# ADharaUTEXAS123007/PhysicsBasedFWI2

Hardware: AMD Instinct MI355X
Metric: grid-cells*timesteps/sec (forward+adjoint gradient pass) (higher is better)
Workload: dtype f32; 1 GPU; elastic_marmousi2_100x300_32shots_3000steps; shots_per_gpu=32, nt=3000, parallelism=shots x1, kernel_family=forward: single launch, 8 slabs/shot; adjoint: single launch, 8 slabs/shot, snapshots=f32, cells=interior

## Files before the change

physicsbasedfwi2_amd/csrc/mifwi_elastic_cluster.h:

```cpp
#pragma once

constexpr int kEcThreads = 512;
constexpr unsigned kEcMaxSpin = 400000;

struct EcParams {
    int nz, nx, ng, gp, pitch;
    unsigned field_stride;
    long long shot_stride;
    int nshot, NW, PL, shot0, shot1;
    int n_first, n_last;
    int W, wl, xr0, wx, fsurf;
    long long psix_shot, psiz_shot;
    const float *mat, *pz, *px;
    float *fields, *psix, *psiz;
    float *S;
    int s_first;
    long long s_step;
    int nsrc, nrec;
    const int *src_cell;
    const float *src_w, *f;
    const int *rec_cell;
    const float *rec_w;
    float *rec_vx, *rec_vz;
    unsigned long long *xbuf;
    int *err;
    int *xcc_tab;
    int dbg, nap;
    FdK K;
#ifdef MIFWI_ABLATIONS
    long long *trace;
#endif
};

#ifdef MIFWI_ABLATIONS
#define EC_STAMP(k)                                                                                        \
    do {                                                                                                   \
        if (p.trace && tr_on && it >= 64 && it < 128 && (t & 63) == 0)                                     \
            p.trace[((it - 64) * 8 + (t >> 6)) * 16 + (k)] = (long long)__builtin_readcyclecounter();      \
    } while (0)
#define EC_LAGGARD()                                                                                       \
    do {                                                                                                   \
        if ((kDbg(p) & 4096) && w == 1 && s == p.shot0 && (it & 63) == 1)                                  \
            for (int z_ = 0; z_ < 3000; ++z_) __builtin_amdgcn_s_sleep(127);                               \
    } while (0)
#else
#define EC_STAMP(k) do { } while (0)
#define EC_LAGGARD() do { } while (0)
#endif

constexpr int kEcRowFields = 6;
constexpr int kEcGr = 5;

__device__ __forceinline__ int ec_rf_field(int rf) { return (rf == 0 || rf == 3 || rf == 4) ? 1 : 0; }
__device__ __forceinline__ int ec_rf_lds_row(int rf, int R)
{
    return rf == 0 || rf == 1 ? R + 2 : rf == 2 ? R + 3 : rf == 3 ? 0 : 1;
}

__device__ __forceinline__ int ec_opaque(int x)
{
    asm volatile("" : "+v"(x));
    return x;
}
__device__ __forceinline__ unsigned ec_opaque(unsigned x)
{
    asm volatile("" : "+v"(x));
    return x;
}
__device__ __forceinline__ int ec_fresh(int &x)
{
    asm volatile("" : "+v"(x));
    return x;
}
__device__ __forceinline__ unsigned ec_fresh(unsigned &x)
{
    asm volatile("" : "+v"(x));
    return x;
}

__device__ __forceinline__ int ec_su(int x)
{
    x = __builtin_amdgcn_readfirstlane(x);
    asm volatile("" : "+s"(x));
    return x;
}
__device__ __forceinline__ unsigned ec_su(unsigned x) { return (unsigned)ec_su((int)x); }

template <class T>
__device__ __forceinline__ T *ec_at(T *base, unsigned byte_off)
{
    return reinterpret_cast<T *>(reinterpret_cast<char *>(base) + byte_off);
}
template <class T>
__device__ __forceinline__ const T *ec_at(const T *base, unsigned byte_off)
{
    return reinterpret_cast<const T *>(reinterpret_cast<const char *>(base) + byte_off);
}

__device__ __forceinline__ void ec_pin(float4 &a, float4 &b, float4 &c, float4 &d)
{
    asm volatile("" : "+v"(a.x), "+v"(a.y), "+v"(a.z), "+v"(a.w), "+v"(b.x), "+v"(b.y), "+v"(b.z), "+v"(b.w),
                      "+v"(c.x), "+v"(c.y), "+v"(c.z), "+v"(c.w), "+v"(d.x), "+v"(d.y), "+v"(d.z), "+v"(d.w));
}
__device__ __forceinline__ void ec_pin(float4 &a, float4 &b)
{
    asm volatile("" : "+v"(a.x), "+v"(a.y), "+v"(a.z), "+v"(a.w), "+v"(b.x), "+v"(b.y), "+v"(b.z), "+v"(b.w));
}
__device__ __forceinline__ void ec_pin(float2 &a, float2 &b, float2 &c, float2 &d)
{
    asm volatile("" : "+v"(a.x), "+v"(a.y), "+v"(b.x), "+v"(b.y), "+v"(c.x), "+v"(c.y), "+v"(d.x), "+v"(d.y));
}

typedef float ec_f2 __attribute__((ext_vector_type(2)));
__device__ __forceinline__ ec_f2 ec_2(float a, float b) { ec_f2 r; r.x = a; r.y = b; return r; }
__device__ __forceinline__ ec_f2 ec_2(const float4 &v, int h) { return h == 0 ? ec_2(v.x, v.y) : ec_2(v.z, v.w); }
__device__ __forceinline__ ec_f2 dfw2(const FdK &K, ec_f2 fm1, ec_f2 f0, ec_f2 f1, ec_f2 f2)
{
    return __builtin_elementwise_fma(ec_2(K.c1, K.c1), f1 - f0, ec_2(K.c2, K.c2) * (f2 - fm1));
}
__device__ __forceinline__ ec_f2 dbw2(const FdK &K, ec_f2 fm2, ec_f2 fm1, ec_f2 f0, ec_f2 f1)
{
    return __builtin_elementwise_fma(ec_2(K.c1, K.c1), f0 - fm1, ec_2(K.c2, K.c2) * (f1 - fm2));
}

__device__ __forceinline__ void ec_drain_vmem() { __builtin_amdgcn_s_waitcnt(0x0f70); }
__device__ __forceinline__ void ec_settle(float &x) { asm volatile("" : "+v"(x)); }

template <bool AG> struct EcScope { static constexpr int value = AG ? __HIP_MEMORY_SCOPE_AGENT : __HIP_MEMORY_SCOPE_WORKGROUP; };

struct EcHandoff {
    unsigned long long *xw;
    unsigned xslot8;
    int gp, ng, NW, w, R, t;
    int rcv_lo[kEcGr];
    unsigned rcv_off[kEcGr];
    int *err;
    bool failed, no_wait;
    int nap;

    __device__ __forceinline__ void init(unsigned long long *xbuf, int s, int NW_, int w_, int R_, int PL, int gp_,
                                         int ng_, int t_, int *err_, bool no_wait_, int nap_, int plane_a)
    {
        nap = nap_;
        gp = gp_; ng = ng_; NW = NW_; w = w_; R = R_; t = t_; err = err_; failed = false; no_wait = no_wait_;
        xslot8 = 8u * kEcRowFields * gp;
        xw = xbuf + ((long long)s * NW + w) * 4 * (kEcRowFields * gp);
#pragma unroll
        for (int k = 0; k < kEcGr; ++k) {
            const int e = t + k * kEcThreads;
            rcv_lo[k] = -1;
            rcv_off[k] = 4u * xslot8;
            if (e < kEcRowFields * gp) {
                const int cq = e % gp, rf = e / gp;
                const int col = 4 * (cq % ng) + cq / ng;
                const bool from_above = rf >= 3;
                if (cq < 4 * ng && !(from_above ? w == 0 : w == NW - 1)) {
                    rcv_lo[k] = ec_rf_lds_row(rf, R) * PL + 4 + col + (ec_rf_field(rf) ? plane_a : 0);
                    rcv_off[k] = 8u * e + (from_above ? 0u : 8u * xslot8);
                }
            }
        }
    }

    struct Pending {
        const unsigned long long *base;
        unsigned long long v[kEcGr];
        __device__ __forceinline__ void clear()
        {
            base = nullptr;
#pragma unroll
            for (int k = 0; k < kEcGr; ++k) v[k] = 0;
        }
    };
    __device__ __forceinline__ void sweep(Pending &q)
    {
#pragma unroll
        for (int k = 0; k < kEcGr; ++k)
            q.v[k] = __hip_atomic_load(ec_at(q.base, ec_fresh(rcv_off[k])), __ATOMIC_RELAXED, __HIP_MEMORY_SCOPE_AGENT);
    }
    __device__ __forceinline__ void request(Pending &q, int kind, int parity)
    {
        const unsigned xs8 = ec_su(xslot8);
        q.base = ec_at(xw, (unsigned)(kind * 2 + parity) * xs8) - 4 * (xs8 / 8);
        sweep(q);
    }
    template <bool EAGER = false, class Dest>
    __device__ __forceinline__ void complete(Pending &q, unsigned epoch, Dest dest)
    {
        int lo[kEcGr];
        unsigned need[kEcGr];
#pragma unroll
        for (int k = 0; k < kEcGr; ++k) { lo[k] = ec_fresh(rcv_lo[k]); need[k] = ~(unsigned)(lo[k] >> 31); }
        for (unsigned spins = 0;; ++spins) {
            unsigned bad = 0;
#pragma unroll
            for (int k = 0; k < kEcGr; ++k) bad |= ((unsigned)(q.v[k] >> 32) ^ epoch) & need[k];
            if (spins == mifwi::kSlowPollPasses && (t & 63) == 0) atomicAdd(err + mifwi::kErrSlow, 1);
            if (bad == 0 || no_wait || failed) break;
            if (spins > kEcMaxSpin ||
                ((spins & 255u) == 255u && __hip_atomic_load(err, __ATOMIC_RELAXED, __HIP_MEMORY_SCOPE_AGENT))) {
                if (spins > kEcMaxSpin) __hip_atomic_store(err, 1, __ATOMIC_RELAXED, __HIP_MEMORY_SCOPE_AGENT);
                failed = true;
                break;
            }
            if (!(EAGER && spins == 0)) mifwi::poll_nap(nap);
            sweep(q);
        }
#pragma unroll
        for (int k = 0; k < kEcGr; ++k)
            if (lo[k] >= 0) dest(lo[k], __uint_as_float((unsigned)q.v[k]));
        ec_drain_vmem();
    }
    template <class Dest>
    __device__ __forceinline__ void receive(int kind, unsigned epoch, int parity, Dest dest)
    {
        Pending q;
        request(q, kind, parity);
        complete(q, epoch, dest);
    }

    template <bool AG>
    __device__ __forceinline__ void publish(int lrw, int gq, int kind, unsigned epoch, int parity, const float4 &b,
                                            const float4 &a) const
    {
        unsigned long long *x = ec_at(xw, (unsigned)(kind * 2 + parity) * ec_su(xslot8));
        const unsigned long long tag = (unsigned long long)epoch << 32;
        const float bv[4] = {b.x, b.y, b.z, b.w}, av[4] = {a.x, a.y, a.z, a.w};
        const unsigned gp8 = 8u * ec_su((unsigned)gp), ng8 = 8u * ec_su((unsigned)ng), gq8 = 8u * gq;
        auto put = [&](int rf, const float (&v)[4]) {
            unsigned o = rf * gp8 + gq8;
#pragma unroll
            for (int k = 0; k < 4; ++k) {
                __hip_atomic_store(ec_at(x, o), tag | __float_as_uint(v[k]), __ATOMIC_RELAXED, EcScope<AG>::value);
                o = ec_opaque(o + ng8);
            }
        };
        const int wq = ec_su(w), Rq = ec_su(R);
        if (wq > 0) {
            if (lrw == 0) { put(0, av); put(1, bv); }
            if (lrw == 1) put(2, bv);
        }
        if (wq < ec_su(NW) - 1) {
            if (lrw == Rq - 2) put(3, av);
            if (lrw == Rq - 1) { put(4, av); put(5, bv); }
        }
    }
};

#ifndef EC_LATE_INTERIOR
#define EC_LATE_INTERIOR 1
#endif
#ifndef EA_PUBLISH_FIRST
#define EA_PUBLISH_FIRST 1
#endif
#ifndef EA_MATS_AHEAD_A
#define EA_MATS_AHEAD_A 0
#endif
#ifndef EA_MATS_AHEAD_C
#define EA_MATS_AHEAD_C 1
#endif
struct EcSlot { int lrw, g, cls; };
__host__ __device__ __forceinline__ EcSlot ec_slot(int v, int R, int ng, int slots)
{
    EcSlot s;
    s.lrw = 0; s.g = 0; s.cls = 0;
#if EC_LATE_INTERIOR
    const int nint = (R > 4 ? R - 4 : 0) * ng, nb = R * ng - nint;
    int b0 = (nint + 63) & ~63;
    if (b0 + nb > slots) b0 = nint;
    if (v < nint) {
        const int ir = v / ng;
        s.lrw = 2 + ir; s.g = v - ir * ng; s.cls = v < kEcThreads ? 1 : 3;
    } else if (v >= b0 && v < b0 + nb) {
        const int bi = v - b0, br = bi / ng;
        s.g = bi - br * ng;
        s.lrw = (R > 4 && br >= 2) ? R - 4 + br : br;
        s.cls = 2;
    }
#else
    if (v < R * ng) {
        s.lrw = v / ng; s.g = v - s.lrw * ng;
        s.cls = (s.lrw >= 2 && s.lrw < R - 2) ? 1 : 2;
    }
#endif
    return s;
}

constexpr int kNbL = 1, kNbR = 2, kNbFirst = 4, kNbLast = 8;
__host__ __device__ __forceinline__ int ec_nb(int v, int R, int ng, int slots)
{
    const EcSlot s = ec_slot(v, R, ng, slots);
    if (s.cls == 0) return 0;
    const int lane = v & 63;
    const bool lv = lane != 0 && ec_slot(v - 1, R, ng, slots).cls == s.cls;
    const bool rv = lane != 63 && ec_slot(v + 1, R, ng, slots).cls == s.cls;
    return (lv ? kNbL : 0) | (rv ? kNbR : 0) | (s.g == 0 ? kNbFirst : 0) | (s.g == ng - 1 ? kNbLast : 0);
}
inline bool ec_xhalo_deal_ok(int R, int ng, int slots)
{
    for (int v = 0; v < slots; ++v) {
        const EcSlot s = ec_slot(v, R, ng, slots);
        if (s.cls == 0) continue;
        const int nb = ec_nb(v, R, ng, slots), lane = v & 63;
        if (!(nb & (kNbL | kNbR))) return false;
        const int lc = lane != 0 ? ec_slot(v - 1, R, ng, slots).cls : 0;
        if (lc >= 2 && s.cls >= 2 && lc != s.cls) return false;
    }
    return true;
}
__device__ __forceinline__ float ec_lane_below(float old, float x)
{
    return __int_as_float(__builtin_amdgcn_update_dpp(__float_as_int(old), __float_as_int(x), 0x138, 0xf, 0xf, false));
}
__device__ __forceinline__ float ec_lane_above(float old, float x)
{
    return __int_as_float(__builtin_amdgcn_update_dpp(__float_as_int(old), __float_as_int(x), 0x130, 0xf, 0xf, false));
}
__host__ __device__ __forceinline__ int ec_xh_word(int nb, int lo_floats)
{
    const int roff = !(nb & kNbL) ? -2 : !(nb & kNbR) ? 4 : -lo_floats;
    return roff * 4 + ((nb & kNbFirst) ? 0 : 2) + ((nb & kNbLast) ? 0 : 1);
}
template <bool XH>
__device__ __forceinline__ void ec_xhalo(const float *q, const float4 &c, const int roff, const unsigned keep_xy,
                                         const unsigned keep_zw, float2 &L, float2 &R)
{
    if (!XH) {
        L = ld2(q - 2); R = ld2(q + 4);
        return;
    }
    const float2 rd = ld2(q + roff);
    const float ez = __uint_as_float(__float_as_uint(c.z) & keep_zw), ew = __uint_as_float(__float_as_uint(c.w) & keep_zw);
    const float ex = __uint_as_float(__float_as_uint(c.x) & keep_xy), ey = __uint_as_float(__float_as_uint(c.y) & keep_xy);
    L.x = ec_lane_below(rd.x, ez); L.y = ec_lane_below(rd.y, ew);
    R.x = ec_lane_above(rd.x, ex); R.y = ec_lane_above(rd.y, ey);
}
__device__ __forceinline__ int ec_xh_roff(int xh) { return xh >> 2; }
__device__ __forceinline__ unsigned ec_xh_keep_xy(int xh) { return (unsigned)((int)((unsigned)xh << 30) >> 31); }
__device__ __forceinline__ unsigned ec_xh_keep_zw(int xh) { return (unsigned)((int)((unsigned)xh << 31) >> 31); }
template <bool XH>
__device__ __forceinline__ void ec_xhalo(const float *q, const float4 &c, const int xh, float2 &L, float2 &R)
{
    ec_xhalo<XH>(q, c, ec_xh_roff(xh), ec_xh_keep_xy(xh), ec_xh_keep_zw(xh), L, R);
}

struct EcGroup {
    int cls;
    int nb;
    int g, j;
    int lo;
    unsigned gcb;
    int xtab, ztab;
    float4 mL, mM, mMu, mBx, mBz;
    float4 s1, s2, s3, s4, s5, s6, s7, s8;
};

__device__ __forceinline__ int ec_plane(int f) { return f == F_VX ? 0 : f == F_VZ ? 1 : f == F_SZZ ? 2 : f == F_SXZ ? 3 : 4; }

__device__ __forceinline__ void ec_stage_tables(float *lpx, float *lpz, const float *px, const float *pz, int gp, int nz,
                                                int r0, int R, int t)
{
    for (int e = t; e < 6 * gp; e += kEcThreads) {
        const int k = e / gp, col = e - k * gp;
        lpx[((col >> 2) * 6 + k) * 4 + (col & 3)] = px[e];
    }
    for (int e = t; e < 8 * R; e += kEcThreads) {
        const int k = e & 7, r = e >> 3;
        lpz[e] = k < 6 ? pz[k * nz + r0 + r] : 0.f;
    }
}
struct EcTabX { float4 v[6]; };
struct EcTabZ { float v[8]; };
__device__ __forceinline__ EcTabX ec_tab_x(const float *lpx, int xtab)
{
    EcTabX r;
#pragma unroll
    for (int k = 0; k < 6; ++k) r.v[k] = ld4(lpx + xtab + 4 * k);
    return r;
}
__device__ __forceinline__ EcTabZ ec_tab_z(const float *lpz, int ztab)
{
    const float4 a = ld4(lpz + ztab);
    const float2 b = ld2(lpz + ztab + 4);
    EcTabZ r;
    r.v[0] = a.x; r.v[1] = a.y; r.v[2] = a.z; r.v[3] = a.w; r.v[4] = b.x; r.v[5] = b.y; r.v[6] = 0.f; r.v[7] = 0.f;
    return r;
}

struct EcCtx {
    float *Lf[5];
    const float *lpx, *lpz;
    int PL, fsurf;
    FdK K;
};

template <bool EDGE, bool XH>
__device__ __forceinline__ void ec_update_v(EcGroup &G, const EcCtx &c, const int lo, const int jq, float4 &S4, float4 &S5,
                                            float4 &o0, float4 &o1)
{
    const int PL = ec_su(c.PL);
    const FdK K = c.K;
    const float *sxx = ec_at(c.Lf[F_SXX], lo), *szz = ec_at(c.Lf[F_SZZ], lo), *sxz = ec_at(c.Lf[F_SXZ], lo);
    const int nb = XH ? ec_fresh(G.nb) : 0;
    float4 cxx = ld4(sxx);
    float4 a2 = ld4(sxz);
    float2 Lxx, Rxx, Lxz, Rxz;
    float4 a0 = ld4(sxz - 2 * PL), a1 = ld4(sxz - PL);
    float4 a3 = ld4(sxz + PL);
    float4 b0 = ld4(szz - PL);
    float4 b1 = ld4(szz), b2 = ld4(szz + PL), b3 = ld4(szz + 2 * PL);
    ec_xhalo<XH>(sxx, cxx, nb, Lxx, Rxx);
    ec_xhalo<XH>(sxz, a2, nb, Lxz, Rxz);
// ... 510 lines not shown
    const unsigned ncell_ = ncell;

    const int par_in = (p.nt - 1 - p.n_first) & 1;
    const float *psi_in = par_in ? p.psiB : p.psiA;
    const int par_out = (p.nt - 1 - (p.n_last - 1)) & 1;
    float *psi_out = par_out ? p.psiB : p.psiA;

    EaGroup G[NG];
    bool slow = false;
#pragma unroll
    for (int q = 0; q < NG; ++q) {
        EaGroup &g = G[q];
        const EcSlot sl = ec_slot(t + q * kEcThreads, R, p.ng, NG * kEcThreads);
        const bool own = sl.cls != 0;
        const int lrw = sl.lrw;
        g.g = sl.g;
        g.j = r0 + lrw;
        g.lo = 4 * ((lrw + 2) * PL + 4 + 4 * g.g);
        g.cls = sl.cls;
        g.nb = XH ? ec_xh_word(ec_nb(t + q * kEcThreads, R, p.ng, NG * kEcThreads), g.lo / 4) : 0;
        g.bxx = g.bzz = g.bxz = g.vx = g.vz = zero4;
        g.a0 = g.a1 = g.a2 = g.a3 = g.a4 = zero4;
        g.S1 = g.S2 = g.S3 = g.S4 = g.S5 = zero4;
        g.xsl = -1; g.zsl = -1; g.src = -1; g.src_wt = 0.f;
        if (own) {
            const unsigned gcc = (unsigned)g.j * p.gp + 4 * g.g;
            const long long o = (long long)(g.j + 2) * p.pitch + 4 + 4 * g.g;
            const float *gf = p.fields + (long long)s * p.shot_stride;
            g.vx = ld4(gf + F_VX * p.field_stride + o); g.vz = ld4(gf + F_VZ * p.field_stride + o);
            g.bxx = ld4(gf + F_SXX * p.field_stride + o); g.bzz = ld4(gf + F_SZZ * p.field_stride + o);
            g.bxz = ld4(gf + F_SXZ * p.field_stride + o);
            const float *ga = p.acc + (long long)s * 5 * ncell + gcc;
            g.a0 = ld4(ga); g.a1 = ld4(ga + ncell); g.a2 = ld4(ga + 2 * (long long)ncell);
            g.a3 = ld4(ga + 3 * (long long)ncell); g.a4 = ld4(ga + 4 * (long long)ncell);
            if (p.W > 0) {
                const int c0 = 4 * g.g;
                int xs_off = -1, zs = -1;
                if (c0 < p.wl) xs_off = c0; else if (c0 >= p.xr0) xs_off = p.wl + (c0 - p.xr0);
                if (g.j < p.W) zs = g.j; else if (g.j >= p.nz - p.W) zs = g.j - (p.nz - 2 * p.W);
                if (xs_off >= 0) {
                    g.xsl = lrw * p.wx + xs_off;
                    const float *qx = psi_in + (long long)s * p.psix_shot + (long long)g.j * p.wx + xs_off;
#pragma unroll
                    for (int k = 0; k < 4; ++k) st4(lxs + k * xsz + g.xsl, ld4(qx + k * xplane));
                }
                if (zs >= 0) {
                    const int zl = (g.j < p.W) ? g.j - r0 : ntop + (g.j - zbot_beg);
                    g.zsl = zl * p.gp + 4 * g.g;
                    const float *qz = psi_in + p.psix_elems + (long long)s * p.psiz_shot + (long long)zs * p.gp + 4 * g.g;
#pragma unroll
                    for (int k = 0; k < 4; ++k) st4(lzs + k * zsz + g.zsl, ld4(qz + k * zplane));
                }
            }
        }
        if (p.grad_f != nullptr)
            for (int e = 0; e < p.nsrc; ++e) {
                const int cell = p.src_cell[(long long)s * p.nsrc + e];
                if (cell < 0) continue;
                const int i0 = cell / p.nx, i1 = cell - i0 * p.nx;
                if (own && i0 == g.j && (i1 >> 2) == g.g) {
                    if (g.src >= 0) slow = true;
                    g.src = (e << 2) | (i1 & 3); g.src_wt = p.src_w[(long long)s * p.nsrc + e];
                }
            }
    }
    slow = __syncthreads_or(slow ? 1 : 0) != 0;
    const bool zero_tap = p.grad_f != nullptr && w == 0 && t < p.nsrc && p.src_cell[(long long)s * p.nsrc + t] < 0;
    const int cnt = p.slab_cnt[s * p.NW + w];
    const bool inj_fast = cnt <= kEcThreads;
    int inj_lo = -1, inj_row = 0, inj_col = 0;
    unsigned inj_id4 = 0;
    float inj_w = 0.f, amp_x = 0.f, amp_z = 0.f;
    if (inj_fast && t < cnt) {
        const int inj_id = p.slab_list[((long long)s * p.NW + w) * p.nrec + t];
        const int cell = p.rec_cell[(long long)s * p.nrec + inj_id];
        const int i0 = cell / p.nx, i1 = cell - i0 * p.nx;
        inj_row = i0 - r0; inj_col = i1;
        inj_lo = (i0 - r0 + 2) * PL + 4 + i1;
        inj_w = p.rec_w[(long long)s * p.nrec + inj_id];
        inj_id4 = 4u * inj_id;
    }

    ec_stage_tables(lpx, lpz, p.px, p.pz, p.gp, p.nz, r0, R, t);
    for (int e = t; e < fsz; e += kEcThreads) { pln[e] = 0.f; pln[fsz + e] = 0.f; pln[2 * fsz + e] = 0.f; pln[3 * fsz + e] = 0.f; }
    int *rowmap = reinterpret_cast<int *>(lzs + 4 * zsz);
    float *rbuf = lzs + 4 * zsz + ((R + 4) & ~3);
    int inj_co = -1;
    bool direct = false;
    if (cnt > 0 && inj_fast && p.rcv_direct) {
        for (int e = t; e <= R; e += kEcThreads) rowmap[e] = 0;
        for (int e = t; e < 2 * kEaRcvRows * PL; e += kEcThreads) rbuf[e] = 0.f;
        __syncthreads();
        if (t < cnt) rowmap[inj_row] = 1;
        __syncthreads();
        if (t == 0) {
            int k = 0;
            for (int r = 0; r < R; ++r) rowmap[r] = rowmap[r] ? k++ : -1;
            rowmap[R] = k;
        }
        __syncthreads();
        direct = rowmap[R] <= kEaRcvRows;
        if (direct) {
            int *ib = reinterpret_cast<int *>(rbuf);
            if (t < cnt) {
                inj_co = rowmap[inj_row] * PL + 4 + inj_col;
                ib[inj_co] = t;
            }
            __syncthreads();
            const int dup = (t < cnt && ib[inj_co] != t) ? 1 : 0;
            direct = __syncthreads_or(dup) == 0;
            if (t < cnt) ib[inj_co] = 0;
            if (!direct) inj_co = -1;
        }
    }
    __syncthreads();

    EcHandoff X;
    X.init(p.xbuf, s, p.NW, w, R, PL, p.gp, p.ng, t, p.err, false, p.nap, fsz);
    const bool do_x = p.NW > 1 && !(kDbg(p) & 1);
    EcHandoff::Pending P;
    auto complete = [&](unsigned epoch) {
        X.complete<EA_EARLY_REQUEST != 0>(P, epoch, [&](int off, float v) { (pln + fsz)[off] = v; });
    };
    auto cell_bytes = [&](int jq, int gq) { return 4u * (unsigned)(jq * p.gp + 4 * gq); };
    const float *S_shot = p.S + (long long)s * 5 * ncell;
    auto request_S = [&](EaGroup &g, int n) {
        if (ec_fresh(g.cls) == 0 || (kDbg(p) & 2)) return;
        const unsigned ncell = ec_su(ncell_);
        const float *Sn = S_shot + (long long)(n - p.s_first) * p.s_step;
        const unsigned gcb = cell_bytes(ec_fresh(g.j), ec_fresh(g.g));
        g.S1 = mifwi::ldnt4(ec_at(Sn, gcb)); g.S2 = mifwi::ldnt4(ec_at(Sn + (long long)ncell, gcb));
        g.S3 = mifwi::ldnt4(ec_at(Sn + 2 * (long long)ncell, gcb));
        g.S4 = mifwi::ldnt4(ec_at(Sn + 3 * (long long)ncell, gcb)); g.S5 = mifwi::ldnt4(ec_at(Sn + 4 * (long long)ncell, gcb));
    };
    auto request_amp = [&](int n) {
        if (ec_fresh(inj_lo) >= 0 && n >= p.n_last) {
            const long long o = ((long long)n * p.nshot + s) * p.nrec;
            amp_x = *ec_at(p.g_vx + o, ec_fresh(inj_id4));
            amp_z = *ec_at(p.g_vz + o, ec_fresh(inj_id4));
        }
    };

    auto mats_a = [&](EaGroup &g, float4 &Ls, float4 &Ms, float4 &mus) {
        const unsigned ncell = ec_su(ncell_);
        const unsigned gcb = cell_bytes(ec_fresh(g.j), ec_fresh(g.g));
        Ls = ld4(ec_at(p.mat + M_L * ncell, gcb)); Ms = ld4(ec_at(p.mat + M_M * ncell, gcb));
        mus = ld4(ec_at(p.mat + M_MU * ncell, gcb));
    };
    auto mats_c = [&](EaGroup &g, float4 &bxs, float4 &bzs) {
        const unsigned ncell = ec_su(ncell_);
        const unsigned gcb = cell_bytes(ec_fresh(g.j), ec_fresh(g.g));
        bxs = ld4(ec_at(p.mat + M_BX * ncell, gcb)); bzs = ld4(ec_at(p.mat + M_BZ * ncell, gcb));
    };
    auto phase_a = [&](EaGroup &g, int n, int it, const int cls, const float4 &Ls, const float4 &Ms, const float4 &mus) {
        const int fsz = ec_su(fsz_), xsz = ec_su(xsz_), zsz = ec_su(zsz_);
        const int lo = ec_fresh(g.lo), gq = ec_fresh(g.g), jq = ec_fresh(g.j);
        const bool top = p.fsurf && jq == 0;
        const float4 bzz = make_float4(top ? 0.f : g.bzz.x, top ? 0.f : g.bzz.y, top ? 0.f : g.bzz.z,
                                       top ? 0.f : g.bzz.w);
        const int src = ec_fresh(g.src);
        if (p.grad_f != nullptr && src >= 0) {
            float *out = p.grad_f + ((long long)n * p.nshot + s) * p.nsrc;
            const float pr[4] = {g.bxx.x + bzz.x, g.bxx.y + bzz.y, g.bxx.z + bzz.z, g.bxx.w + bzz.w};
            if (!slow) {
                float v = 0.f;
#pragma unroll
                for (int c = 0; c < 4; ++c)
                    if (c == (src & 3)) v = pr[c];
                *ec_at(out, 4u * (unsigned)(src >> 2)) = fmaf(g.src_wt, v, 0.f);
            } else {
                for (int e = 0; e < p.nsrc; ++e) {
                    const int cell = p.src_cell[(long long)s * p.nsrc + e];
                    if (cell < 0) continue;
                    const int i0 = cell / p.nx, i1 = cell - i0 * p.nx;
                    if (i0 != jq || (i1 >> 2) != gq) continue;
                    float v = 0.f;
#pragma unroll
                    for (int c = 0; c < 4; ++c)
                        if (c == (i1 & 3)) v = pr[c];
                    out[e] = fmaf(p.src_w[(long long)s * p.nsrc + e], v, 0.f);
                }
            }
        }
        float e1[4], e2[4], e3[4], e4[4];
#pragma unroll
        for (int c = 0; c < 4; ++c) {
            e1[c] = fmaf(comp(Ms, c), comp(g.bxx, c), comp(Ls, c) * comp(bzz, c));
            e2[c] = fmaf(comp(Ls, c), comp(g.bxx, c), comp(Ms, c) * comp(bzz, c));
            e3[c] = comp(mus, c) * comp(g.bxz, c);
            e4[c] = e3[c];
        }
        const int xsl = ec_fresh(g.xsl), zsl = ec_fresh(g.zsl);
        if (xsl >= 0) {
            const EcTabX T = ec_tab_x(lpx, 24 * gq);
            float *sl = lxs + xsl;
            const float4 s5 = ld4(sl + 2 * xsz), s8 = ld4(sl + 3 * xsz);
            float n5[4], n8[4];
#pragma unroll
            for (int c = 0; c < 4; ++c) {
                e1[c] = pmlT(comp(s5, c), comp(T.v[PA], c), comp(T.v[PB], c), comp(T.v[PK], c), e1[c], n5[c]);
                e4[c] = pmlT(comp(s8, c), comp(T.v[PAH], c), comp(T.v[PBH], c), comp(T.v[PKH], c), e4[c], n8[c]);
            }
            st4(sl + 2 * xsz, make_float4(n5[0], n5[1], n5[2], n5[3]));
            st4(sl + 3 * xsz, make_float4(n8[0], n8[1], n8[2], n8[3]));
        }
        if (zsl >= 0) {
            const EcTabZ Z = ec_tab_z(lpz, 8 * (jq - r0));
            float *sl = lzs + zsl;
            const float4 s6 = ld4(sl + 2 * zsz), s7 = ld4(sl + 3 * zsz);
            float n6[4], n7[4];
#pragma unroll
            for (int c = 0; c < 4; ++c) {
                e2[c] = pmlT(comp(s6, c), Z.v[PA], Z.v[PB], Z.v[PK], e2[c], n6[c]);
                e3[c] = pmlT(comp(s7, c), Z.v[PAH], Z.v[PBH], Z.v[PKH], e3[c], n7[c]);
            }
            st4(sl + 2 * zsz, make_float4(n6[0], n6[1], n6[2], n6[3]));
            st4(sl + 3 * zsz, make_float4(n7[0], n7[1], n7[2], n7[3]));
        }
        const float4 E2 = make_float4(e2[0], e2[1], e2[2], e2[3]), E3 = make_float4(e3[0], e3[1], e3[2], e3[3]);
        st4(ec_at(pln, lo), make_float4(e1[0], e1[1], e1[2], e1[3]));
        st4(ec_at(pln + fsz, lo), E2);
        st4(ec_at(pln + 2 * fsz, lo), E3);
        st4(ec_at(pln + 3 * fsz, lo), make_float4(e4[0], e4[1], e4[2], e4[3]));
        if (do_x && cls == 2) X.template publish<AG>(jq - r0, gq, 0, (unsigned)(2 * it + 1), it & 1, E2, E3);
    };
    auto phase_b = [&](EaGroup &g) {
        const int fsz = ec_su(fsz_), PL = ec_su(PL_);
        const int lo = ec_fresh(g.lo), gq = ec_fresh(g.g);
        const float *E1 = ec_at(pln, lo), *E2 = ec_at(pln + fsz, lo), *E3 = ec_at(pln + 2 * fsz, lo),
                    *E4 = ec_at(pln + 3 * fsz, lo);
        const int nb = XH ? ec_fresh(g.nb) : 0;
        const float4 c1 = ld4(E1);
        const float4 c4 = ld4(E4);
        const float4 t0 = ld4(E3 - 2 * PL), t1 = ld4(E3 - PL), t2 = ld4(E3), t3 = ld4(E3 + PL);
        const float4 u0 = ld4(E2 - PL), u1 = ld4(E2), u2 = ld4(E2 + PL), u3 = ld4(E2 + 2 * PL);
        float2 L1, R1, L4, R4;
        ec_xhalo<XH>(E1, c1, nb, L1, R1);
        ec_xhalo<XH>(E4, c4, nb, L4, R4);
        const float x1[8] = {L1.x, L1.y, c1.x, c1.y, c1.z, c1.w, R1.x, R1.y};
        const float x4[8] = {L4.x, L4.y, c4.x, c4.y, c4.z, c4.w, R4.x, R4.y};
        float nvx[4], nvz[4];
#pragma unroll
        for (int h = 0; h < 4; h += 2) {
            const ec_f2 dx1 = dfw2(K, ec_2(x1[h + 1], x1[h + 2]), ec_2(x1[h + 2], x1[h + 3]), ec_2(x1[h + 3], x1[h + 4]),
                                   ec_2(x1[h + 4], x1[h + 5]));
            const ec_f2 dz3 = dbw2(K, ec_2(t0, h), ec_2(t1, h), ec_2(t2, h), ec_2(t3, h));
            const ec_f2 dz2 = dfw2(K, ec_2(u0, h), ec_2(u1, h), ec_2(u2, h), ec_2(u3, h));
            const ec_f2 dx4 = dbw2(K, ec_2(x4[h], x4[h + 1]), ec_2(x4[h + 1], x4[h + 2]), ec_2(x4[h + 2], x4[h + 3]),
                                   ec_2(x4[h + 3], x4[h + 4]));
            const ec_f2 vx2 = ec_2(g.vx, h) - (dx1 + dz3), vz2 = ec_2(g.vz, h) - (dz2 + dx4);
            nvx[h] = vx2.x; nvx[h + 1] = vx2.y; nvz[h] = vz2.x; nvz[h + 1] = vz2.y;
        }
        if (ec_su(p.nx & 3)) {
#pragma unroll
            for (int c = 1; c < 4; ++c)
                if (4 * gq + c >= p.nx) { nvx[c] = 0.f; nvz[c] = 0.f; }
        }
        g.vx = make_float4(nvx[0], nvx[1], nvx[2], nvx[3]);
        g.vz = make_float4(nvz[0], nvz[1], nvz[2], nvz[3]);
    };
    auto phase_c = [&](EaGroup &g, int it, const int cls, const float4 &bxs, const float4 &bzs) {
        const int fsz = ec_su(fsz_), xsz = ec_su(xsz_), zsz = ec_su(zsz_);
        const int lo = ec_fresh(g.lo), gq = ec_fresh(g.g), jq = ec_fresh(g.j);
        float d1[4], d2[4], d3[4], d4[4];
#pragma unroll
        for (int c = 0; c < 4; ++c) {
            d1[c] = comp(bxs, c) * comp(g.vx, c); d2[c] = d1[c];
            d3[c] = comp(bzs, c) * comp(g.vz, c); d4[c] = d3[c];
        }
        const int xsl = ec_fresh(g.xsl), zsl = ec_fresh(g.zsl);
        if (xsl >= 0) {
            const EcTabX T = ec_tab_x(lpx, 24 * gq);
            float *sl = lxs + xsl;
            const float4 s1 = ld4(sl), s3 = ld4(sl + xsz);
            float n1[4], n3[4];
#pragma unroll
            for (int c = 0; c < 4; ++c) {
                d1[c] = pmlT(comp(s1, c), comp(T.v[PAH], c), comp(T.v[PBH], c), comp(T.v[PKH], c), d1[c], n1[c]);
                d3[c] = pmlT(comp(s3, c), comp(T.v[PA], c), comp(T.v[PB], c), comp(T.v[PK], c), d3[c], n3[c]);
            }
            st4(sl, make_float4(n1[0], n1[1], n1[2], n1[3]));
            st4(sl + xsz, make_float4(n3[0], n3[1], n3[2], n3[3]));
        }
        if (zsl >= 0) {
            const EcTabZ Z = ec_tab_z(lpz, 8 * (jq - r0));
            float *sl = lzs + zsl;
            const float4 s2 = ld4(sl), s4 = ld4(sl + zsz);
            float n2[4], n4[4];
#pragma unroll
            for (int c = 0; c < 4; ++c) {
                d2[c] = pmlT(comp(s2, c), Z.v[PA], Z.v[PB], Z.v[PK], d2[c], n2[c]);
                d4[c] = pmlT(comp(s4, c), Z.v[PAH], Z.v[PBH], Z.v[PKH], d4[c], n4[c]);
            }
            st4(sl, make_float4(n2[0], n2[1], n2[2], n2[3]));
            st4(sl + zsz, make_float4(n4[0], n4[1], n4[2], n4[3]));
        }
        const float4 D2 = make_float4(d2[0], d2[1], d2[2], d2[3]), D4 = make_float4(d4[0], d4[1], d4[2], d4[3]);
        st4(ec_at(pln, lo), make_float4(d1[0], d1[1], d1[2], d1[3]));
        st4(ec_at(pln + fsz, lo), D2);
        st4(ec_at(pln + 2 * fsz, lo), D4);
        st4(ec_at(pln + 3 * fsz, lo), make_float4(d3[0], d3[1], d3[2], d3[3]));
        if (do_x && cls == 2) X.template publish<AG>(jq - r0, gq, 1, (unsigned)(2 * it + 2), it & 1, D2, D4);
        const bool top = p.fsurf && jq == 0;
        const float4 bzz = make_float4(top ? 0.f : g.bzz.x, top ? 0.f : g.bzz.y, top ? 0.f : g.bzz.z,
                                       top ? 0.f : g.bzz.w);
#define EA_ACC3(dst, a, b, c_, d) dst = fmaf(a, b, fmaf(c_, d, dst))
        EA_ACC3(g.a1.x, g.S1.x, g.bxx.x, g.S2.x, bzz.x); EA_ACC3(g.a1.y, g.S1.y, g.bxx.y, g.S2.y, bzz.y);
        EA_ACC3(g.a1.z, g.S1.z, g.bxx.z, g.S2.z, bzz.z); EA_ACC3(g.a1.w, g.S1.w, g.bxx.w, g.S2.w, bzz.w);
        EA_ACC3(g.a0.x, g.S2.x, g.bxx.x, g.S1.x, bzz.x); EA_ACC3(g.a0.y, g.S2.y, g.bxx.y, g.S1.y, bzz.y);
        EA_ACC3(g.a0.z, g.S2.z, g.bxx.z, g.S1.z, bzz.z); EA_ACC3(g.a0.w, g.S2.w, g.bxx.w, g.S1.w, bzz.w);
#undef EA_ACC3
        g.a2.x = fmaf(g.S3.x, g.bxz.x, g.a2.x); g.a2.y = fmaf(g.S3.y, g.bxz.y, g.a2.y);
        g.a2.z = fmaf(g.S3.z, g.bxz.z, g.a2.z); g.a2.w = fmaf(g.S3.w, g.bxz.w, g.a2.w);
        g.a3.x = fmaf(g.S4.x, g.vx.x, g.a3.x); g.a3.y = fmaf(g.S4.y, g.vx.y, g.a3.y);
        g.a3.z = fmaf(g.S4.z, g.vx.z, g.a3.z); g.a3.w = fmaf(g.S4.w, g.vx.w, g.a3.w);
        g.a4.x = fmaf(g.S5.x, g.vz.x, g.a4.x); g.a4.y = fmaf(g.S5.y, g.vz.y, g.a4.y);
        g.a4.z = fmaf(g.S5.z, g.vz.z, g.a4.z); g.a4.w = fmaf(g.S5.w, g.vz.w, g.a4.w);
    };
    auto phase_d = [&](EaGroup &g, const bool edge) {
        const int fsz = ec_su(fsz_), PL = ec_su(PL_);
        const int lo = ec_fresh(g.lo), gq = ec_fresh(g.g);
        const float *D1 = ec_at(pln, lo), *D2 = ec_at(pln + fsz, lo), *D4 = ec_at(pln + 2 * fsz, lo),
                    *D3 = ec_at(pln + 3 * fsz, lo);
        const int nb = XH ? ec_fresh(g.nb) : 0;
        const float4 c1 = ld4(D1);
        const float4 c3 = ld4(D3);
        const float4 u0 = ld4(D2 - PL), u1 = ld4(D2), u2 = ld4(D2 + PL), u3 = ld4(D2 + 2 * PL);
        const float4 t0 = ld4(D4 - 2 * PL), t1 = ld4(D4 - PL), t2 = ld4(D4), t3 = ld4(D4 + PL);
        float2 L1, R1, L3, R3;
        ec_xhalo<XH>(D1, c1, nb, L1, R1);
        ec_xhalo<XH>(D3, c3, nb, L3, R3);
        const float x1[8] = {L1.x, L1.y, c1.x, c1.y, c1.z, c1.w, R1.x, R1.y};
        const float x3[8] = {L3.x, L3.y, c3.x, c3.y, c3.z, c3.w, R3.x, R3.y};
        float nxx[4], nzz[4], nxz[4];
#pragma unroll
        for (int h = 0; h < 4; h += 2) {
            const ec_f2 dx1 = dbw2(K, ec_2(x1[h], x1[h + 1]), ec_2(x1[h + 1], x1[h + 2]), ec_2(x1[h + 2], x1[h + 3]),
                                   ec_2(x1[h + 3], x1[h + 4]));
            const ec_f2 dz2 = dfw2(K, ec_2(u0, h), ec_2(u1, h), ec_2(u2, h), ec_2(u3, h));
            const ec_f2 dx3 = dfw2(K, ec_2(x3[h + 1], x3[h + 2]), ec_2(x3[h + 2], x3[h + 3]), ec_2(x3[h + 3], x3[h + 4]),
                                   ec_2(x3[h + 4], x3[h + 5]));
            const ec_f2 dz4 = dbw2(K, ec_2(t0, h), ec_2(t1, h), ec_2(t2, h), ec_2(t3, h));
            const ec_f2 xx2 = ec_2(g.bxx, h) - dx1, xz2 = ec_2(g.bxz, h) - (dz2 + dx3), zz2 = ec_2(g.bzz, h) - dz4;
            nxx[h] = xx2.x; nxx[h + 1] = xx2.y; nxz[h] = xz2.x; nxz[h + 1] = xz2.y; nzz[h] = zz2.x; nzz[h + 1] = zz2.y;
        }
        if (edge && p.fsurf) {
            const int jq = ec_fresh(g.j);
            if (jq < 2) {
                const float4 r0d2 = ld4(pln + fsz + 2 * PL + 4 + 4 * gq), r1d2 = ld4(pln + fsz + 3 * PL + 4 + 4 * gq);
                const float4 r0d4 = ld4(pln + 2 * fsz + 2 * PL + 4 + 4 * gq);
#pragma unroll
                for (int c = 0; c < 4; ++c) {
                    if (jq == 0) nxz[c] = nxz[c] + fmaf(K.c1, comp(r0d2, c), K.c2 * comp(r1d2, c));
                    else { nxz[c] = nxz[c] + K.c2 * comp(r0d2, c); nzz[c] = nzz[c] + K.c2 * comp(r0d4, c); }
                }
            }
        }
        if (ec_su(p.nx & 3)) {
#pragma unroll
            for (int c = 1; c < 4; ++c)
                if (4 * gq + c >= p.nx) { nxx[c] = 0.f; nxz[c] = 0.f; nzz[c] = 0.f; }
        }
        g.bxx = make_float4(nxx[0], nxx[1], nxx[2], nxx[3]);
        g.bzz = make_float4(nzz[0], nzz[1], nzz[2], nzz[3]);
        g.bxz = make_float4(nxz[0], nxz[1], nxz[2], nxz[3]);
    };

    const int nsteps = p.n_first - p.n_last + 1;
#ifdef MIFWI_ABLATIONS
    const bool tr_on = w == (((kDbg(p) >> 8) & 15) ? ((kDbg(p) >> 8) & 15) - 1 : p.NW / 2) && s == p.shot0;
#endif
    ec_drain_vmem();
#pragma unroll
    for (int q = 0; q < NG; ++q) request_S(G[q], p.n_first);
    request_amp(p.n_first);
    for (int it = 0; it < nsteps; ++it) {
        const int n = p.n_first - it;
        EC_LAGGARD();
        EC_STAMP(0);
        float4 mL[NG], mM[NG], mMu[NG];
#if EA_MATS_AHEAD_A
#pragma unroll
        for (int qq = 0; qq < NG; ++qq) {
            const int q = EA_PUBLISH_FIRST ? NG - 1 - qq : qq;
            if (ec_fresh(G[q].cls) != 0) mats_a(G[q], mL[q], mM[q], mMu[q]);
        }
        __builtin_amdgcn_sched_barrier(0);
#endif
#pragma unroll
        for (int qq = 0; qq < NG; ++qq) {
            const int q = EA_PUBLISH_FIRST ? NG - 1 - qq : qq;
            const int cls = ec_fresh(G[q].cls);
#if !EA_MATS_AHEAD_A
            if (cls != 0) mats_a(G[q], mL[q], mM[q], mMu[q]);
#endif
            if (cls != 0) phase_a(G[q], n, it, cls, mL[q], mM[q], mMu[q]);
            __builtin_amdgcn_sched_barrier(0);
        }
        if (p.grad_f != nullptr && w == 0) {
            if (zero_tap) (p.grad_f + ((long long)n * p.nshot + s) * p.nsrc)[t] = 0.f;
            for (int e = ec_opaque(t) + kEcThreads; e < p.nsrc; e += kEcThreads)
                if (p.src_cell[(long long)s * p.nsrc + e] < 0) p.grad_f[((long long)n * p.nshot + s) * p.nsrc + e] = 0.f;
        }
        if (direct) {
            const int co = ec_fresh(inj_co);
            if (co >= 0) {
                rbuf[co] = inj_w * amp_x;
                rbuf[kEaRcvRows * PL_ + co] = inj_w * amp_z;
            }
        }
        EC_STAMP(1);
        __syncthreads();
        EC_STAMP(2);
        if (it > 0) {
#pragma unroll
            for (int q = 0; q < NG; ++q)
                if ((q == 0 ? EA_S0 : EA_S1) == 1) request_S(G[q], n);
        }
        if (EA_EARLY_REQUEST && do_x) X.request(P, 0, it & 1);
#pragma unroll
        for (int q = 0; q < NG; ++q) {
            if ((!EC_LATE_INTERIOR || q == 0) && ec_fresh(G[q].cls) == 1) phase_b(G[q]);
            __builtin_amdgcn_sched_barrier(0);
        }
        EC_STAMP(3);
        if (do_x) {
            if (!EA_EARLY_REQUEST) X.request(P, 0, it & 1);
            complete((unsigned)(2 * it + 1));
        }
        EC_STAMP(4);
        __syncthreads();
        EC_STAMP(5);
#ifndef MIFWI_EA_NO_SETTLE
        ec_settle(amp_x);
        ec_settle(amp_z);
#endif
        if (it > 0) {
#pragma unroll
            for (int q = 0; q < NG; ++q)
                if ((q == 0 ? EA_S0 : EA_S1) == 2) request_S(G[q], n);
        }
#pragma unroll
        for (int q = 0; q < NG; ++q) {
            if (ec_fresh(G[q].cls) >= 2) phase_b(G[q]);
            __builtin_amdgcn_sched_barrier(0);
        }
        EC_STAMP(6);
        __syncthreads();
        EC_STAMP(7);
        if (direct) {
#pragma unroll
            for (int q = 0; q < NG; ++q)
                if (ec_fresh(G[q].cls) != 0) {
                    const int rr = rowmap[ec_fresh(G[q].j) - r0];
                    if (rr >= 0) {
                        const float *b = rbuf + rr * PL_ + 4 + 4 * ec_fresh(G[q].g);
                        const float4 ix = ld4(b), iz = ld4(b + kEaRcvRows * PL_);
                        G[q].vx = make_float4(G[q].vx.x + ix.x, G[q].vx.y + ix.y, G[q].vx.z + ix.z, G[q].vx.w + ix.w);
                        G[q].vz = make_float4(G[q].vz.x + iz.x, G[q].vz.y + iz.y, G[q].vz.z + iz.z, G[q].vz.w + iz.w);
                    }
                }
        } else if (cnt > 0) {
#pragma unroll
            for (int q = 0; q < NG; ++q)
                if (ec_fresh(G[q].cls) != 0) { st4(ec_at(pln, ec_fresh(G[q].lo)), zero4); st4(ec_at(pln + fsz, ec_fresh(G[q].lo)), zero4); }
            __syncthreads();
            if (inj_fast) {
                const int il = ec_fresh(inj_lo);
                if (il >= 0) {
                    atomicAdd(pln + il, inj_w * amp_x);
                    atomicAdd(pln + fsz + il, inj_w * amp_z);
                }
            } else {
                const int *lst = p.slab_list + ((long long)s * p.NW + w) * p.nrec;
                for (int e = ec_opaque(t); e < cnt; e += kEcThreads) {
                    const int id = lst[e];
                    const int cell = p.rec_cell[(long long)s * p.nrec + id];
                    const int i0 = cell / p.nx, i1 = cell - i0 * p.nx;
                    const float ww = p.rec_w[(long long)s * p.nrec + id];
                    const long long o = ((long long)n * p.nshot + s) * p.nrec + id;
                    atomicAdd(pln + (i0 - r0 + 2) * PL + 4 + i1, ww * p.g_vx[o]);
                    atomicAdd(pln + fsz + (i0 - r0 + 2) * PL + 4 + i1, ww * p.g_vz[o]);
                }
            }
            __syncthreads();
#pragma unroll
            for (int q = 0; q < NG; ++q)
                if (ec_fresh(G[q].cls) != 0) {
                    const float4 ix = ld4(ec_at(pln, ec_fresh(G[q].lo))), iz = ld4(ec_at(pln + fsz, ec_fresh(G[q].lo)));
                    G[q].vx = make_float4(G[q].vx.x + ix.x, G[q].vx.y + ix.y, G[q].vx.z + ix.z, G[q].vx.w + ix.w);
                    G[q].vz = make_float4(G[q].vz.x + iz.x, G[q].vz.y + iz.y, G[q].vz.z + iz.z, G[q].vz.w + iz.w);
                }
        }
        EC_STAMP(8);
        float4 mBx[NG], mBz[NG];
#if EA_MATS_AHEAD_C
#pragma unroll
        for (int qq = 0; qq < NG; ++qq) {
            const int q = EA_PUBLISH_FIRST ? NG - 1 - qq : qq;
            if (ec_fresh(G[q].cls) != 0) mats_c(G[q], mBx[q], mBz[q]);
        }
        __builtin_amdgcn_sched_barrier(0);
#endif
#pragma unroll
        for (int qq = 0; qq < NG; ++qq) {
            const int q = EA_PUBLISH_FIRST ? NG - 1 - qq : qq;
            const int cls = ec_fresh(G[q].cls);
#if !EA_MATS_AHEAD_C
            if (cls != 0) mats_c(G[q], mBx[q], mBz[q]);
#endif
            if (cls != 0) phase_c(G[q], it, cls, mBx[q], mBz[q]);
            __builtin_amdgcn_sched_barrier(0);
        }
        EC_STAMP(9);
        __syncthreads();
        EC_STAMP(10);
        if (EA_EARLY_REQUEST && do_x) X.request(P, 1, it & 1);
#pragma unroll
        for (int q = 0; q < NG; ++q) {
            if ((!EC_LATE_INTERIOR || q == 0) && ec_fresh(G[q].cls) == 1) phase_d(G[q], false);
            __builtin_amdgcn_sched_barrier(0);
        }
        EC_STAMP(11);
        if (do_x) {
            if (!EA_EARLY_REQUEST) X.request(P, 1, it & 1);
            complete((unsigned)(2 * it + 2));
        }
        EC_STAMP(12);
        if (!do_x) ec_drain_vmem();
        if (it + 1 < nsteps) {
#pragma unroll
            for (int q = 0; q < NG; ++q)
                if ((q == 0 ? EA_S0 : EA_S1) == 0) request_S(G[q], n - 1);
        }
        if (cnt > 0) request_amp(n - 1);
        EC_STAMP(13);
        __syncthreads();
        EC_STAMP(14);
#pragma unroll
        for (int q = 0; q < NG; ++q) {
            const int cls = ec_fresh(G[q].cls);
            if (cls == 2) phase_d(G[q], true);
            else if (q > 0 && cls == 3) phase_d(G[q], false);
            __builtin_amdgcn_sched_barrier(0);
        }
        EC_STAMP(15);
        if ((it & 31) == 31 || it == nsteps - 1) {
            if (__syncthreads_or(X.failed ? 1 : 0)) {
                if (t == 0) __hip_atomic_store(p.err, 1, __ATOMIC_RELAXED, __HIP_MEMORY_SCOPE_AGENT);
                break;
            }
        } else {
            __syncthreads();
        }
    }

    float *gf = p.fields + (long long)s * p.shot_stride;
#pragma unroll
    for (int q = 0; q < NG; ++q) {
        const EaGroup &g = G[q];
        if (g.cls == 0) continue;
        const long long o = (long long)(g.j + 2) * p.pitch + 4 + 4 * g.g;
        st4(gf + F_VX * p.field_stride + o, g.vx); st4(gf + F_VZ * p.field_stride + o, g.vz);
        st4(gf + F_SXX * p.field_stride + o, g.bxx); st4(gf + F_SZZ * p.field_stride + o, g.bzz);
        st4(gf + F_SXZ * p.field_stride + o, g.bxz);
        const unsigned gcc = (unsigned)g.j * p.gp + 4 * g.g;
        float *ga = p.acc + (long long)s * 5 * ncell + gcc;
        st4(ga, g.a0); st4(ga + ncell, g.a1); st4(ga + 2 * (long long)ncell, g.a2);
        st4(ga + 3 * (long long)ncell, g.a3); st4(ga + 4 * (long long)ncell, g.a4);
        if (g.xsl >= 0) {
            const int xs_off = g.xsl - (g.j - r0) * p.wx;
            float *qx = psi_out + (long long)s * p.psix_shot + (long long)g.j * p.wx + xs_off;
#pragma unroll
            for (int k = 0; k < 4; ++k) st4(qx + k * xplane, ld4(lxs + k * xsz + g.xsl));
        }
        if (g.zsl >= 0) {
            const int zs = (g.j < p.W) ? g.j : g.j - (p.nz - 2 * p.W);
            float *qz = psi_out + p.psix_elems + (long long)s * p.psiz_shot + (long long)zs * p.gp + 4 * g.g;
#pragma unroll
            for (int k = 0; k < 4; ++k) st4(qz + k * zplane, ld4(lzs + k * zsz + g.zsl));
        }
    }
}
```

Before: 74450 Mcells*steps/s.

## Prefetch adjoint material coefficients across phases and time steps

In the adjoint kernel, the L/M/mu material loads for the first group are now issued at the end of the previous time step, and the second group's loads are issued in the middle of phase A, after the first group's stress products are computed. The bx/bz loads for phase C are moved before the preceding barrier. The aim is to hide global-memory latency for the material reads behind other work. The cost is extra live registers and explicit vmem drains, which could reduce occupancy or serialise other outstanding loads.

```diff
diff --git a/physicsbasedfwi2_amd/csrc/mifwi_elastic_cluster.h b/physicsbasedfwi2_amd/csrc/mifwi_elastic_cluster.h
--- a/physicsbasedfwi2_amd/csrc/mifwi_elastic_cluster.h
+++ b/physicsbasedfwi2_amd/csrc/mifwi_elastic_cluster.h
@@ -125,6 +125,10 @@
 
 __device__ __forceinline__ void ec_drain_vmem() { __builtin_amdgcn_s_waitcnt(0x0f70); }
 __device__ __forceinline__ void ec_settle(float &x) { asm volatile("" : "+v"(x)); }
+__device__ __forceinline__ void ec_forget(float4 &a)
+{
+    asm volatile("" : "=v"(a.x), "=v"(a.y), "=v"(a.z), "=v"(a.w));
+}
 
 template <bool AG> struct EcScope { static constexpr int value = AG ? __HIP_MEMORY_SCOPE_AGENT : __HIP_MEMORY_SCOPE_WORKGROUP; };
 
@@ -253,11 +257,8 @@
 #ifndef EA_PUBLISH_FIRST
 #define EA_PUBLISH_FIRST 1
 #endif
-#ifndef EA_MATS_AHEAD_A
-#define EA_MATS_AHEAD_A 0
-#endif
-#ifndef EA_MATS_AHEAD_C
-#define EA_MATS_AHEAD_C 1
+#ifndef EA_MATS_PREFETCH
+#define EA_MATS_PREFETCH 1
 #endif
 struct EcSlot { int lrw, g, cls; };
 __host__ __device__ __forceinline__ EcSlot ec_slot(int v, int R, int ng, int slots)
@@ -1074,12 +1075,25 @@
         const unsigned gcb = cell_bytes(ec_fresh(g.j), ec_fresh(g.g));
         bxs = ld4(ec_at(p.mat + M_BX * ncell, gcb)); bzs = ld4(ec_at(p.mat + M_BZ * ncell, gcb));
     };
-    auto phase_a = [&](EaGroup &g, int n, int it, const int cls, const float4 &Ls, const float4 &Ms, const float4 &mus) {
+    auto phase_a = [&](EaGroup &g, int n, int it, const int cls, const float4 &Ls, const float4 &Ms, const float4 &mus,
+                       auto &&between) {
         const int fsz = ec_su(fsz_), xsz = ec_su(xsz_), zsz = ec_su(zsz_);
         const int lo = ec_fresh(g.lo), gq = ec_fresh(g.g), jq = ec_fresh(g.j);
         const bool top = p.fsurf && jq == 0;
         const float4 bzz = make_float4(top ? 0.f : g.bzz.x, top ? 0.f : g.bzz.y, top ? 0.f : g.bzz.z,
                                        top ? 0.f : g.bzz.w);
+        float e1[4], e2[4], e3[4], e4[4];
+#pragma unroll
+        for (int c = 0; c < 4; ++c) {
+            e1[c] = fmaf(comp(Ms, c), comp(g.bxx, c), comp(Ls, c) * comp(bzz, c));
+            e2[c] = fmaf(comp(Ls, c), comp(g.bxx, c), comp(Ms, c) * comp(bzz, c));
+            e3[c] = comp(mus, c) * comp(g.bxz, c);
+        }
+        asm volatile("" : "+v"(e1[0]), "+v"(e1[1]), "+v"(e1[2]), "+v"(e1[3]), "+v"(e2[0]), "+v"(e2[1]), "+v"(e2[2]),
+                          "+v"(e2[3]), "+v"(e3[0]), "+v"(e3[1]), "+v"(e3[2]), "+v"(e3[3]));
+#pragma unroll
+        for (int c = 0; c < 4; ++c) e4[c] = e3[c];
+        between();
         const int src = ec_fresh(g.src);
         if (p.grad_f != nullptr && src >= 0) {
             float *out = p.grad_f + ((long long)n * p.nshot + s) * p.nsrc;
@@ -1103,14 +1117,6 @@
                     out[e] = fmaf(p.src_w[(long long)s * p.nsrc + e], v, 0.f);
                 }
             }
-        }
-        float e1[4], e2[4], e3[4], e4[4];
-#pragma unroll
-        for (int c = 0; c < 4; ++c) {
-            e1[c] = fmaf(comp(Ms, c), comp(g.bxx, c), comp(Ls, c) * comp(bzz, c));
-            e2[c] = fmaf(comp(Ls, c), comp(g.bxx, c), comp(Ms, c) * comp(bzz, c));
-            e3[c] = comp(mus, c) * comp(g.bxz, c);
-            e4[c] = e3[c];
         }
         const int xsl = ec_fresh(g.xsl), zsl = ec_fresh(g.zsl);
         if (xsl >= 0) {
@@ -1296,31 +1302,51 @@
 #pragma unroll
     for (int q = 0; q < NG; ++q) request_S(G[q], p.n_first);
     request_amp(p.n_first);
+    constexpr int qa0 = EA_PUBLISH_FIRST ? NG - 1 : 0;
+#if EA_MATS_PREFETCH
+    float4 aL = zero4, aM = zero4, aMu = zero4;
+    if (ec_fresh(G[qa0].cls) != 0) mats_a(G[qa0], aL, aM, aMu);
+#endif
     for (int it = 0; it < nsteps; ++it) {
         const int n = p.n_first - it;
         EC_LAGGARD();
         EC_STAMP(0);
-        float4 mL[NG], mM[NG], mMu[NG];
-#if EA_MATS_AHEAD_A
-#pragma unroll
-        for (int qq = 0; qq < NG; ++qq) {
-            const int q = EA_PUBLISH_FIRST ? NG - 1 - qq : qq;
-            if (ec_fresh(G[q].cls) != 0) mats_a(G[q], mL[q], mM[q], mMu[q]);
-        }
-        __builtin_amdgcn_sched_barrier(0);
-#endif
+#if EA_MATS_PREFETCH
+        {
+            constexpr int qa1 = NG - 1 - qa0;
+            float4 bL, bM, bMu;
+            auto ask_second = [&]() {
+                if (NG > 1) {
+                    __builtin_amdgcn_sched_barrier(0);
+                    if (ec_fresh(G[qa1].cls) != 0) mats_a(G[qa1], bL, bM, bMu);
+                    __builtin_amdgcn_sched_barrier(0);
+                }
+            };
+            ec_drain_vmem();
+            const int cls0 = ec_fresh(G[qa0].cls);
+            if (cls0 != 0) phase_a(G[qa0], n, it, cls0, aL, aM, aMu, ask_second);
+            else ask_second();
+            __builtin_amdgcn_sched_barrier(0);
+            if (NG > 1) {
+                ec_drain_vmem();
+                const int cls1 = ec_fresh(G[qa1].cls);
+                if (cls1 != 0) phase_a(G[qa1], n, it, cls1, bL, bM, bMu, [] {});
+                __builtin_amdgcn_sched_barrier(0);
+            }
+        }
+#else
 #pragma unroll
         for (int qq = 0; qq < NG; ++qq) {
             const int q = EA_PUBLISH_FIRST ? NG - 1 - qq : qq;
             const int cls = ec_fresh(G[q].cls);
-#if !EA_MATS_AHEAD_A
-            if (cls != 0) mats_a(G[q], mL[q], mM[q], mMu[q]);
-#endif
-            if (cls != 0) phase_a(G[q], n, it, cls, mL[q], mM[q], mMu[q]);
+            float4 mL, mM, mMu;
+            if (cls != 0) mats_a(G[q], mL, mM, mMu);
+            if (cls != 0) phase_a(G[q], n, it, cls, mL, mM, mMu, [] {});
             __builtin_amdgcn_sched_barrier(0);
         }
+#endif
         if (p.grad_f != nullptr && w == 0) {
-            if (zero_tap) (p.grad_f + ((long long)n * p.nshot + s) * p.nsrc)[t] = 0.f;
+            if (zero_tap) *ec_at(p.grad_f + ((long long)n * p.nshot + s) * p.nsrc, 4u * (unsigned)ec_opaque(t)) = 0.f;
             for (int e = ec_opaque(t) + kEcThreads; e < p.nsrc; e += kEcThreads)
                 if (p.src_cell[(long long)s * p.nsrc + e] < 0) p.grad_f[((long long)n * p.nshot + s) * p.nsrc + e] = 0.f;
         }
@@ -1367,6 +1393,15 @@
             if (ec_fresh(G[q].cls) >= 2) phase_b(G[q]);
             __builtin_amdgcn_sched_barrier(0);
         }
+        float4 mBx[NG], mBz[NG];
+#if EA_MATS_PREFETCH
+#pragma unroll
+        for (int qq = 0; qq < NG; ++qq) {
+            const int q = EA_PUBLISH_FIRST ? NG - 1 - qq : qq;
+            if (ec_fresh(G[q].cls) != 0) mats_c(G[q], mBx[q], mBz[q]);
+        }
+        __builtin_amdgcn_sched_barrier(0);
+#endif
         EC_STAMP(6);
         __syncthreads();
         EC_STAMP(7);
@@ -1415,22 +1450,20 @@
                 }
         }
         EC_STAMP(8);
-        float4 mBx[NG], mBz[NG];
-#if EA_MATS_AHEAD_C
+#if !EA_MATS_PREFETCH
 #pragma unroll
         for (int qq = 0; qq < NG; ++qq) {
             const int q = EA_PUBLISH_FIRST ? NG - 1 - qq : qq;
             if (ec_fresh(G[q].cls) != 0) mats_c(G[q], mBx[q], mBz[q]);
         }
         __builtin_amdgcn_sched_barrier(0);
+#else
+        ec_drain_vmem();
 #endif
 #pragma unroll
         for (int qq = 0; qq < NG; ++qq) {
             const int q = EA_PUBLISH_FIRST ? NG - 1 - qq : qq;
             const int cls = ec_fresh(G[q].cls);
-#if !EA_MATS_AHEAD_C
-            if (cls != 0) mats_c(G[q], mBx[q], mBz[q]);
-#endif
             if (cls != 0) phase_c(G[q], it, cls, mBx[q], mBz[q]);
             __builtin_amdgcn_sched_barrier(0);
         }
@@ -1467,6 +1500,11 @@
             __builtin_amdgcn_sched_barrier(0);
         }
         EC_STAMP(15);
+#if EA_MATS_PREFETCH
+        ec_forget(aL); ec_forget(aM); ec_forget(aMu);
+        if (it + 1 < nsteps && ec_fresh(G[qa0].cls) != 0) mats_a(G[qa0], aL, aM, aMu);
+        __builtin_amdgcn_sched_barrier(0);
+#endif
         if ((it & 31) == 31 || it == nsteps - 1) {
             if (__syncthreads_or(X.failed ? 1 : 0)) {
                 if (t == 0) __hip_atomic_store(p.err, 1, __ATOMIC_RELAXED, __HIP_MEMORY_SCOPE_AGENT);
```

After: 72620 Mcells*steps/s. -2.5%, worse.
